# ViacheslavDanilov/oct_segmentation

Hardware: AMD Instinct MI355X
Metric: OCT frames/sec (704x704, bf16) fwd+bwd (higher is better)
Workload: dtype bf16; 1 GPU; unetplusplus/resnet101 1-class 704x704, batch 16/GPU, fwd+Dice+bwd+allreduce+Adam; global_batch=16, parallelism=dp1

## Files before the change

include/octseg.h:

```cpp
#ifndef OCTSEG_H
#define OCTSEG_H
#include <stddef.h>
#include <stdint.h>

#ifdef __cplusplus
extern "C" {
#endif

typedef enum {
  OCTSEG_OK = 0,
  OCTSEG_BAD_SHAPE = -1,
  OCTSEG_BAD_DTYPE = -2,
  OCTSEG_UNSUPPORTED_ARCH = -3,
  OCTSEG_HIP_ERROR = -4,
  OCTSEG_BAD_ARG = -5
} octseg_status;

typedef enum { OCTSEG_F32 = 0, OCTSEG_BF16 = 1, OCTSEG_F16 = 2 } octseg_dtype;

typedef struct {
  const char* arch;
  const char* encoder;
  int classes;
  int batch, height, width;
// ... 176 lines not shown

int octseg_resize_pil_u8(const uint8_t* src, int S, int H, int W, int C, uint8_t* tmp, uint8_t* dst, int oh, int ow, const int* xbounds,
                         const int* xkk, int xksize, const int* ybounds, const int* ykk, int yksize, void* stream);

int octseg_plan_set_frozen_bn(octseg_plan* plan, int on);
int octseg_plan_cam_target(const octseg_plan* plan, size_t* act_off, size_t* grad_off, int* dims);
int octseg_net_backward_seeded(octseg_plan* plan, const float* params, void* workspace, const float* dlogits, void* stream);
size_t octseg_cam_scratch_bytes(int N, int h, int w, int K);
int octseg_cam_maps(int dtype, const void* A, const void* G, int N, int h, int w, int K, int method, int S, void* scratch, float* maps,
                    float threshold, uint8_t* bin, const uint8_t* gt, int gt_h, int gt_w, const int* row_index, const int* col_index, int* counts,
                    const float* frames, const uint8_t* jet_bgr, double image_weight, uint8_t* overlay, void* stream);

int octseg_cam_overlay(const float* maps, const float* frames, const uint8_t* jet_bgr, int N, int S, double image_weight, uint8_t* overlay,
                       void* scratch, void* stream);

typedef enum { OCTSEG_LOSS_DICE = 0, OCTSEG_LOSS_BCE = 1, OCTSEG_LOSS_DICE_BCE = 2 } octseg_loss_kind;
int octseg_plan_set_loss(octseg_plan* plan, int kind);

int octseg_dice_forward(octseg_plan* plan, void* workspace, const float* logits, const float* target,
                        float* loss, long long* stats, void* stream);

int octseg_net_backward(octseg_plan* plan, const float* params, float* grads, void* workspace,
                        const float* logits, const float* target, float grad_scale, void* stream);

int octseg_net_train_step(octseg_plan* plan, const float* params, float* grads, float* buffers, void* workspace, const float* image,
                          const float* target, float* logits, float* loss, long long* stats, int normalize, const float* mean,
                          const float* stdv, float grad_scale, void* stream);
int octseg_plan_set_train_graph(octseg_plan* plan, int enable);

typedef void (*octseg_slice_cb)(void* user, int slice, size_t begin, size_t end);
int octseg_net_backward_sliced(octseg_plan* plan, const float* params, float* grads, void* workspace, const float* logits,
                               const float* target, float grad_scale, void* stream, int nslices, void* comm_stream,
                               octseg_slice_cb cb, void* user);

int octseg_optim_step(int kind, float* params, const float* grads, float* state_m, float* state_v,
                      size_t numel, float lr, float weight_decay, int step, float grad_scale,
                      void* stream);

int octseg_set_deterministic(int on);

int octseg_debug_set_stamp(unsigned long long* dev_buf);
int octseg_debug_set_serial(int on);

size_t octseg_conv2d_scratch_bytes(int dtype, int N, int H, int W, int Cin, int Cout, int R, int S);
int octseg_conv2d_forward(int dtype, const void* x, const float* w, const float* bias, void* y, int N,
                          int H, int W, int Cin, int Cout, int R, int S, int stride, int pad,
                          int transposed, void* scratch, void* stream);
int octseg_conv2d_backward_data(int dtype, const void* dy, const float* w, void* dx, int N, int H, int W,
                                int Cin, int Cout, int R, int S, int stride, int pad, int transposed,
                                void* scratch, void* stream);
int octseg_conv2d_backward_weight(int dtype, const void* x, const void* dy, float* dw, int N, int H,
                                  int W, int Cin, int Cout, int R, int S, int stride, int pad,
                                  int transposed, void* stream);

#define OCTSEG_CONV_MAX_SRC 5
typedef enum { OCTSEG_CONV_FORWARD = 0, OCTSEG_CONV_BACKWARD_DATA = 1, OCTSEG_CONV_BACKWARD_WEIGHT = 2 } octseg_conv_mode;
typedef enum { OCTSEG_ROUTE_THIN = 0, OCTSEG_ROUTE_GEMM1X1, OCTSEG_ROUTE_CONV3X3P, OCTSEG_ROUTE_MFMA16, OCTSEG_ROUTE_MFMA11,
               OCTSEG_ROUTE_MFMA_WIDEN,
               OCTSEG_ROUTE_MFMA11_MASKED, OCTSEG_ROUTE_MFMA16_MASKED } octseg_conv_route;
typedef enum { OCTSEG_WROUTE_THIN = 0, OCTSEG_WROUTE_WGRAD1X1, OCTSEG_WROUTE_CONVT16, OCTSEG_WROUTE_MFMA } octseg_wgrad_route;
typedef struct {
  const void* ptr; const float* scale; const float* shift;
  int C, H, W, up, relu;
} octseg_conv_src;
typedef struct { void* ptr; int accum, pool; } octseg_conv_dst;
typedef struct {
// ... 119 lines not shown
```

oct_segmentation_amd/_lib.py:

```python
import ctypes as C
import os

def set_hw_queues_for_collectives():
    os.environ.setdefault('GPU_MAX_HW_QUEUES', '8')


if int(os.environ.get('WORLD_SIZE', '1') or 1) > 1:
    set_hw_queues_for_collectives()

import torch

_HERE = os.path.dirname(os.path.abspath(__file__))
LIB_PATH = os.path.join(_HERE, 'liboctseg_hip.so')

F32, BF16, F16 = 0, 1, 2
P_CONV, P_CONVT, P_STEM, P_VEC = 0, 1, 2, 3
OPT_KINDS = {'SGD': 0, 'Adam': 1, 'RMSprop': 2, 'RAdam': 3}


class NetDesc(C.Structure):
    _fields_ = [('arch', C.c_char_p), ('encoder', C.c_char_p), ('classes', C.c_int), ('batch', C.c_int),
                ('height', C.c_int), ('width', C.c_int), ('dtype', C.c_int)]


# ... 117 lines not shown
    'octseg_pair_distance_counts': (C.c_int, [_P, _P] + [C.c_int] * 5 + [_P] + [C.c_int] * 3 + [_P, C.c_size_t, _P, _P, _P]),
    'octseg_pair_distance_keys': (C.c_int, [_P, _P] + [C.c_int] * 5 + [_P] + [C.c_int] * 3 + [_P, C.c_size_t, C.c_longlong, _P, _P, C.c_longlong,
                                            _P, _P]),
    'octseg_pair_distance_min': (C.c_int, [_P, _P] + [C.c_int] * 5 + [_P] + [C.c_int] * 3 + [_P, C.c_size_t, _P, _P]),
    'octseg_volume_distance_scratch_bytes': (C.c_size_t, [C.c_int] * 7),
    'octseg_volume_boundary': (C.c_int, [_P] + [C.c_int] * 4 + [_P, C.c_size_t, _P, _P]),
    'octseg_volume_distance': (C.c_int, [_P] + [C.c_int] * 6 + [_P, C.c_size_t, _P, _P]),
    'octseg_volume_pair_distance_counts': (C.c_int, [_P, _P] + [C.c_int] * 5 + [_P] + [C.c_int] * 3 + [_P, C.c_size_t, _P, _P, _P]),
    'octseg_volume_pair_distance_keys': (C.c_int, [_P, _P] + [C.c_int] * 5 + [_P] + [C.c_int] * 4 + [_P, C.c_size_t, C.c_longlong, _P, _P,
                                                   C.c_longlong, _P, _P]),
    'octseg_volume_pair_distance_min': (C.c_int, [_P, _P] + [C.c_int] * 5 + [_P] + [C.c_int] * 4 + [_P, C.c_size_t, _P, _P]),
    'octseg_signed_distance_scratch_bytes': (C.c_size_t, [C.c_int] * 4),
    'octseg_stack_signed_distance': (C.c_int, [_P] + [C.c_int] * 4 + [_P, C.c_size_t, _P, _P]),
    'octseg_signed_blend': (C.c_int, [_P] + [C.c_int] * 4 + [_P, C.c_int, _P, C.c_int, _P, _P]),
    'octseg_skeleton_scratch_bytes': (C.c_size_t, [C.c_int] * 4),
    'octseg_stack_skeleton': (C.c_int, [_P] + [C.c_int] * 5 + [_P, C.c_size_t, _P, _P, _P]),
    'octseg_prune_scratch_bytes': (C.c_size_t, [C.c_int] * 4),
    'octseg_stack_prune': (C.c_int, [_P] + [C.c_int] * 7 + [_P, C.c_size_t, _P, _P, _P]),
    'octseg_volume_normalize': (C.c_int, [_P] + [C.c_int] * 6 + [_P, _P, _P]),
    'octseg_resize_pil_u8': (C.c_int, [_P] + [C.c_int] * 4 + [_P, _P, C.c_int, C.c_int, _P, _P, C.c_int, _P, _P, C.c_int, _P]),
    'octseg_plan_set_frozen_bn': (C.c_int, [_P, C.c_int]),
    'octseg_plan_cam_target': (C.c_int, [_P, C.POINTER(C.c_size_t), C.POINTER(C.c_size_t), C.POINTER(C.c_int)]),
    'octseg_net_backward_seeded': (C.c_int, [_P, _P, _P, _P, _P]),
    'octseg_cam_scratch_bytes': (C.c_size_t, [C.c_int] * 4),
    'octseg_cam_maps': (C.c_int, [C.c_int, _P, _P] + [C.c_int] * 6 + [_P, _P, C.c_float, _P, _P, C.c_int, C.c_int, _P, _P, _P, _P, _P, C.c_double, _P, _P]),
    'octseg_cam_overlay': (C.c_int, [_P, _P, _P, C.c_int, C.c_int, C.c_double, _P, _P, _P]),
    'octseg_plan_set_loss': (C.c_int, [_P, C.c_int]),
    'octseg_dice_forward': (C.c_int, [_P, _P, _P, _P, _P, _P, _P]),
    'octseg_net_backward': (C.c_int, [_P, _P, _P, _P, _P, _P, C.c_float, _P]),
    'octseg_net_train_step': (C.c_int, [_P, _P, _P, _P, _P, _P, _P, _P, _P, _P, C.c_int, C.POINTER(C.c_float), C.POINTER(C.c_float),
                                        C.c_float, _P]),
    'octseg_plan_set_train_graph': (C.c_int, [_P, C.c_int]),
    'octseg_net_backward_sliced': (C.c_int, [_P, _P, _P, _P, _P, _P, C.c_float, _P, C.c_int, _P, SLICE_CB, _P]),
    'octseg_optim_step': (C.c_int, [C.c_int, _P, _P, _P, _P, C.c_size_t, C.c_float, C.c_float, C.c_int, C.c_float, _P]),
    'octseg_set_deterministic': (C.c_int, [C.c_int]),
    'octseg_debug_set_stamp': (C.c_int, [_P]),
    'octseg_debug_set_serial': (C.c_int, [C.c_int]),
    'octseg_conv2d_scratch_bytes': (C.c_size_t, [C.c_int] * 8),
    'octseg_conv2d_forward': (C.c_int, [C.c_int, _P, _P, _P, _P] + [C.c_int] * 10 + [_P, _P]),
    'octseg_conv2d_backward_data': (C.c_int, [C.c_int, _P, _P, _P] + [C.c_int] * 10 + [_P, _P]),
    'octseg_conv2d_backward_weight': (C.c_int, [C.c_int, _P, _P, _P] + [C.c_int] * 10 + [_P]),
    'octseg_conv_layer_op': (C.c_int, [C.c_int, C.c_int, C.POINTER(ConvLayerDesc), _P]),
    'octseg_conv_layer_route': (C.c_int, [C.c_int, C.c_int, C.POINTER(ConvLayerDesc), C.POINTER(C.c_int), C.POINTER(C.c_int)]),
    'octseg_conv_layer_slab_rows': (C.c_int, [C.c_int, C.POINTER(ConvLayerDesc), C.POINTER(C.c_int)]),
    'octseg_tied_layer_op': (C.c_int, [C.c_int, C.c_int, C.POINTER(ConvLayerDesc), C.c_int, _P]),
    'octseg_tied_layer_route': (C.c_int, [C.c_int, C.c_int, C.POINTER(ConvLayerDesc), C.c_int, C.POINTER(C.c_int), C.POINTER(C.c_int)]),
    'octseg_tied_layer_scratch_bytes': (C.c_size_t, [C.c_int, C.POINTER(ConvLayerDesc)]),
    'octseg_side_wgs': (C.c_int, []),
    'octseg_stem_op': (C.c_int, [C.c_int, C.c_int, C.POINTER(StemDesc), _P]),
    'octseg_stem_slab_rows': (C.c_int, [C.c_int] * 3),
    'octseg_sweep_op': (C.c_int, [C.c_int, C.c_int, C.POINTER(_P), C.c_int, C.POINTER(C.c_longlong), C.c_int, C.POINTER(C.c_double), C.c_int, _P]),
    'octseg_fpa_scratch_floats': (C.c_size_t, [C.c_int] * 3),
    'octseg_fpa_gscratch_floats': (C.c_size_t, [C.c_int] * 3),
    'octseg_fpa_uu_offset': (C.c_size_t, [C.c_int] * 3),
    'octseg_fpa_op': (C.c_int, [C.c_int, C.c_int, C.POINTER(FpaDesc), _P]),
    'octseg_pab_op': (C.c_int, [C.c_int, C.c_int, C.POINTER(PabDesc), _P]),
}

_lib = None


def lib():
    global _lib
    if _lib is None:
        if not os.path.exists(LIB_PATH):
            raise RuntimeError(
# ... 27 lines not shown
```

oct_segmentation_amd/csrc/api.cpp:

```cpp
#include "plan_internal.h"

#include <cctype>

using namespace octseg;
using namespace octseg::detail;

static std::string lower(const char* s) {
  std::string r(s ? s : "");
  for (auto& c : r) c = (char)tolower((unsigned char)c);
  return r;
}

template <class Outside, class Body>
static int graph_call(octseg_plan* p, bool train, bool same_key, hipGraphExec_t& exec, int& seen, hipStream_t st, Outside&& outside, Body&& body) {
  if (!same_key) {
    if (exec) { (void)hipGraphExecDestroy(exec); exec = nullptr; }
    seen = 0;
  }
  if (const int rc = outside()) return rc;
  auto replay = [&]() -> int { HIPCHK(hipGraphLaunch(exec, st)); if (train) p->packed_valid = false; return OCTSEG_OK; };
  if (exec) return replay();
  if (seen++ == 0) return body();
  if (train) p->packed_valid = false;
  hipGraph_t g = nullptr;
// ... 17 lines not shown
int octseg_version(void) { return 100; }
const char* octseg_last_error(void) { return g_err.c_str(); }

int octseg_plan_create(const octseg_net_desc* d, octseg_plan** out) {
  if (!d || !out) return fail(OCTSEG_BAD_ARG, "null argument");
  *out = nullptr;
  if (d->dtype != OCTSEG_F32 && d->dtype != OCTSEG_BF16 && d->dtype != OCTSEG_F16) return fail(OCTSEG_BAD_DTYPE, "dtype must be f32, bf16 or f16");
  if (d->height <= 0 || d->width <= 0 || d->height % 32 != 0 || d->width % 32 != 0) {
    char buf[256];
    snprintf(buf, sizeof buf, "Wrong input shape height=%d, width=%d. Expected image height and width divisible by 32.",
             d->height, d->width);
    return fail(OCTSEG_BAD_SHAPE, buf);
  }
  if (d->batch <= 0 || d->classes <= 0 || d->classes > 16) return fail(OCTSEG_BAD_SHAPE, "batch > 0 and 1 <= classes <= 16 required");
  const std::string enc = lower(d->encoder);
  if (enc != "resnet18" && enc != "resnet34" && enc != "resnet50" && enc != "resnet101" && enc != "resnet152" && enc != "timm-regnetx_002" &&
      enc != "timm-regnetx_064" && enc != "timm-regnety_120" && enc != "efficientnet-b0" && enc != "efficientnet-b5" && enc != "efficientnet-b7")
    return fail(OCTSEG_UNSUPPORTED_ARCH, "unknown encoder '" + enc + "' (resnet18 | resnet34 | resnet50 | resnet101 | resnet152 | timm-regnetx_002 | timm-regnetx_064 | timm-regnety_120 | efficientnet-b0 | efficientnet-b5 | efficientnet-b7)");
  octseg_plan* P = new octseg_plan();
  P->arch = lower(d->arch); P->encoder = enc; P->classes = d->classes;
  P->B = d->batch; P->H = d->height; P->W = d->width; P->dtype = d->dtype;
  const int rc = build_plan(P);
  if (rc) { delete P; return rc; }
  *out = P;
  return OCTSEG_OK;
}
int octseg_plan_destroy(octseg_plan* p) {
  if (p) {
    if (p->side) (void)hipStreamDestroy(p->side);
    if (p->side_bwd) (void)hipStreamDestroy(p->side_bwd);
    if (p->ev_fork) (void)hipEventDestroy(p->ev_fork);
    if (p->ev_join) (void)hipEventDestroy(p->ev_join);
    if (p->ev_slice) (void)hipEventDestroy(p->ev_slice);
    if (p->graph_exec) (void)hipGraphExecDestroy(p->graph_exec);
    if (p->tgraph_exec) (void)hipGraphExecDestroy(p->tgraph_exec);
  }
  delete p;
  return OCTSEG_OK;
}
size_t octseg_plan_workspace_bytes(const octseg_plan* p) { return p ? p->ws_bytes : 0; }
size_t octseg_plan_param_numel(const octseg_plan* p) { return p ? p->param_numel : 0; }
size_t octseg_plan_buffer_numel(const octseg_plan* p) { return p ? p->buffer_numel : 0; }
int octseg_plan_num_params(const octseg_plan* p) { return p ? (int)p->params.size() : 0; }
int octseg_plan_num_bn(const octseg_plan* p) { return p ? (int)p->bns.size() : 0; }
double octseg_plan_fwd_macs(const octseg_plan* p) { return p ? p->fwd_macs : 0.0; }
int octseg_plan_exec_macs(const octseg_plan* p, double* out3) {
  if (p == nullptr || out3 == nullptr) return OCTSEG_BAD_ARG;
  for (int k = 0; k < 3; ++k) out3[k] = p->exec_macs[k];
  return OCTSEG_OK;
}

int octseg_plan_param_info(const octseg_plan* p, int i, octseg_param_info* o) {
  if (!p || !o || i < 0 || i >= (int)p->params.size()) return fail(OCTSEG_BAD_ARG, "param index out of range");
  const ParamInfo& q = p->params[i];
  memset(o, 0, sizeof(*o));
  snprintf(o->name, sizeof o->name, "%s", q.name.c_str());
  o->kind = q.kind; o->R = q.R; o->S = q.S; o->O = q.O; o->I = q.I; o->KP = q.KP; o->offset = q.off; o->numel = q.numel;
  return OCTSEG_OK;
}
int octseg_plan_bn_info(const octseg_plan* p, int i, octseg_bn_info* o) {
  if (!p || !o || i < 0 || i >= (int)p->bns.size()) return fail(OCTSEG_BAD_ARG, "bn index out of range");
  const BNInfo& b = p->bns[i];
  memset(o, 0, sizeof(*o));
  snprintf(o->name, sizeof o->name, "%s", b.name.c_str());
  o->C = b.C; o->mean_offset = b.rm_off; o->var_offset = b.rv_off;
  return OCTSEG_OK;
// ... 366 lines not shown
  if (!p) return fail(OCTSEG_BAD_ARG, "null argument");
  if (kind < LOSS_DICE || kind > LOSS_DICE_BCE) return fail(OCTSEG_BAD_ARG, "loss kind must be 0 (dice), 1 (bce) or 2 (dice + bce)");
  if (kind != p->loss_kind && p->tgraph_exec) { (void)hipGraphExecDestroy(p->tgraph_exec); p->tgraph_exec = nullptr; p->tgraph_seen = 0; }
  p->loss_kind = kind;
  return OCTSEG_OK;
}
int octseg_plan_set_drop_connect(octseg_plan* p, const float* factors_dev) {
  if (!p) return fail(OCTSEG_BAD_ARG, "null argument");
  p->drop_connect = factors_dev;
  return OCTSEG_OK;
}
int octseg_plan_num_drop_connect(const octseg_plan* p) { return p ? (int)p->dc_rates.size() : 0; }
float octseg_plan_drop_connect_rate(const octseg_plan* p, int i) { return (p && i >= 0 && i < (int)p->dc_rates.size()) ? p->dc_rates[i] : -1.f; }
int octseg_plan_set_train_graph(octseg_plan* p, int enable) {
  if (!p) return fail(OCTSEG_BAD_ARG, "null argument");
  p->tgraph_enabled = enable != 0;
  if (!enable && p->tgraph_exec) { (void)hipGraphExecDestroy(p->tgraph_exec); p->tgraph_exec = nullptr; p->tgraph_seen = 0; }
  return OCTSEG_OK;
}

int octseg_net_backward_sliced(octseg_plan* p, const float* params, float* grads, void* workspace, const float* logits,
                               const float* target, float grad_scale, void* stream, int nslices, void* comm_stream,
                               octseg_slice_cb cb, void* user) {
  if (!p || !params || !grads || !workspace || !logits || !target || !cb) return fail(OCTSEG_BAD_ARG, "null argument");
  if (nslices < 1 || nslices > 64) return fail(OCTSEG_BAD_ARG, "1 <= nslices <= 64 required");
  if (p->dtype == OCTSEG_F16) return fail(OCTSEG_BAD_DTYPE, "f16 is a serving dtype: no backward");
  if (!comm_stream || comm_stream == stream) return fail(OCTSEG_BAD_ARG, "comm_stream must be a stream of its own");
  Exec E{p, params, grads, nullptr, (char*)workspace, (hipStream_t)stream, 1};
  SliceCtx S;
  S.n = nslices; S.comm = (hipStream_t)comm_stream; S.cb = cb; S.user = user;
  return run_backward(E, logits, target, grad_scale, &S);
}

int octseg_optim_step(int kind, float* params, const float* grads, float* m, float* v, size_t numel, float lr,
                      float wd, int step, float grad_scale, void* stream) {
  if (!params || !grads) return fail(OCTSEG_BAD_ARG, "null argument");
  if (kind < 0 || kind > 3) return fail(OCTSEG_BAD_ARG, "optimizer kind must be 0..3");
  if ((kind == 1 || kind == 3) && (!m || !v)) return fail(OCTSEG_BAD_ARG, "Adam/RAdam need both state arenas");
  if (kind == 2 && !v) return fail(OCTSEG_BAD_ARG, "RMSprop needs the second-moment arena");
  OptArgs a;
  memset(&a, 0, sizeof(a));
  a.p = params; a.g = grads; a.m = m; a.v = v; a.n = numel; a.kind = kind; a.lr = lr; a.wd = wd;
  a.beta1 = 0.9f; a.beta2 = 0.999f; a.eps = 1e-8f; a.alpha = 0.99f; a.momentum = 0.f; a.step = step; a.grad_scale = grad_scale;
  HIPCHK(launch_optim_step(a, (hipStream_t)stream));
  return OCTSEG_OK;
}

static unsigned long long* g_stamp = nullptr;
static bool g_serial = false;
int octseg_debug_set_stamp(unsigned long long* dev_buf) { g_stamp = dev_buf; return OCTSEG_OK; }
int octseg_debug_set_serial(int on) { g_serial = on != 0; g_prof_hbm = g_serial; return OCTSEG_OK; }

size_t octseg_conv2d_scratch_bytes(int dtype, int N, int H, int W, int Cin, int Cout, int R, int S) {
  (void)N; (void)H; (void)W;
  const size_t esz = dtype_size(dtype);
  const size_t rows_f = ((size_t)Cout + 127) / 128 * 128, k_f = ((size_t)Cin + 63) / 64 * 64;
  const size_t rows_d = ((size_t)Cin + 127) / 128 * 128, k_d = ((size_t)Cout + 63) / 64 * 64;
  return align_up((size_t)R * S * rows_f * k_f * esz) + align_up((size_t)R * S * rows_d * k_d * esz);
}

int octseg_conv2d_forward(int dtype, const void* x, const float* w, const float* bias, void* y, int N, int H, int W,
                          int Cin, int Cout, int R, int S, int stride, int pad, int transposed, void* scratch, void* stream) {
  if (!geom_ok(dtype, Cin, Cout, R, S, stride, transposed)) return fail(OCTSEG_BAD_SHAPE, "unsupported conv geometry");
  hipStream_t st = (hipStream_t)stream;
  const Geom g = op_geom(N, H, W, Cin, Cout, R, S, stride, pad, transposed);
  std::vector<ConvArgs> la;
// ... 82 lines not shown
```

oct_segmentation_amd/csrc/plan.h:

```cpp
#pragma once
#include <string>
#include <vector>
#include "common.h"
#include "kernels.h"
#include "../../include/octseg.h"

namespace octseg {

struct TensorInfo {
  int N, H, W, C;
  size_t off;
  size_t goff;
  bool need_grad;
  bool external;
  size_t mask_off = 0;
  int grad_alias = -1;
};

struct Value {
  int t = -1;
  int bn = -1;
};

struct ParamInfo {
// ... 59 lines not shown
              OP_DW,
              OP_GAP,
              OP_BCAST,
              OP_DROPE,
              OP_UPB,
              OP_BINPOOL,
              OP_RESIZE,
              OP_RELU,
              OP_DROP2D,
              OP_MOSAIC,
              OP_STATS,
              OP_SEGATE,
              OP_DWG,
              OP_BNX,
              OP_SEFC,
              OP_PAB,
              OP_FPA,
              OP_ADD };
struct Op {
  OpKind kind;
  int conv = -1;
  int bn = -1;
  Value y, res;
  int post = -1;
  bool relu = true;
  int in = -1, out = -1;
  int lane = 0;
  int gn = -1, up = 1;
  int ins[4] = {-1, -1, -1, -1};
  int dwp = -1, oc0 = 0, wc0 = 0;
  bool dw_first = true;
  size_t aux_off = 0;
  bool conv_bn = false;
};

}

struct octseg_plan {
  std::string arch, encoder;
  int classes, B, H, W, dtype;
  std::vector<octseg::TensorInfo> tensors;
  std::vector<octseg::ParamInfo> params;
  std::vector<octseg::BNInfo> bns;
  std::vector<octseg::ConvLayer> convs;
  std::vector<octseg::GNInfo> gns;
  std::vector<octseg::Op> ops;
  int head_up = 1;
  size_t z4_off = 0, dz4_off = 0;
  const float* stem_image = nullptr; int stem_normalize = 0; float stem_mean[3] = {0, 0, 0}, stem_std[3] = {1, 1, 1};
  const float* dropout_keep = nullptr;
  float dropout_p = 0.2f;
  size_t param_numel = 0, buffer_numel = 0;
  size_t ws_bytes = 0;
  size_t act_begin = 0, act_end = 0, grad_begin = 0, grad_end = 0;
  size_t slab_off = 0, slab_bytes = 0;
  bool has_lanes = false;
  size_t fin_part_off = 0, fin_cnt_off = 0;
  size_t pool_idx_off = 0;
  size_t tmp_off = 0, tmp_bytes = 0;
  size_t se_part_off = 0;
  int stem_pad = 3;
  const float* drop_connect = nullptr;
  std::vector<float> dc_rates;
  std::string run_error;
  struct { int w[6], b[6], bn[6]; int pool = -1; size_t scratch_off = 0, gscratch_off = 0; } fpa;
  size_t dlogits_off = 0;
  bool frozen_bn = false;
  int loss_kind = 0;
  size_t dice_off = 0;
  int col_tensor = -1;
  int stem_k = 7;
  int dlogits_C = 16;
  double fwd_macs = 0;
  double exec_macs[3] = {0, 0, 0};
  size_t tie_scratch_off = 0;
  bool packed_valid = false;
  bool packed_fold = false;
  const void* packed_buffers = nullptr;
  const void* packed_ws = nullptr;
  const void* packed_params = nullptr;
  std::vector<octseg::PackJob> pack_jobs;
  std::vector<unsigned long long> pack_prefix;
  unsigned long long pack_total = 0;
  size_t pack_tab_off = 0, pack_prefix_off = 0;
  const void* pack_tab_ws = nullptr;
  std::vector<octseg::BnEvalJob> bn_jobs;
  std::vector<unsigned> bn_prefix;
  unsigned bn_total = 0;
  size_t bn_tab_off = 0, bn_prefix_off = 0;
  hipStream_t side = nullptr;
  hipStream_t side_bwd = nullptr;
  hipEvent_t ev_fork = nullptr, ev_join = nullptr, ev_slice = nullptr;
  bool graph_enabled = false;
  int graph_seen = 0;
  hipGraphExec_t graph_exec = nullptr;
  struct GraphKey {
    const void* params; const void* buffers; const void* ws; const void* image; const void* logits; const void* stream;
    int normalize; float mean[3], stdv[3];
    bool operator==(const GraphKey& o) const {
      return params == o.params && buffers == o.buffers && ws == o.ws && image == o.image && logits == o.logits &&
             stream == o.stream && normalize == o.normalize && mean[0] == o.mean[0] && mean[1] == o.mean[1] &&
             mean[2] == o.mean[2] && stdv[0] == o.stdv[0] && stdv[1] == o.stdv[1] && stdv[2] == o.stdv[2];
    }
  } graph_key{};
  bool tgraph_enabled = false;
  int tgraph_seen = 0;
  hipGraphExec_t tgraph_exec = nullptr;
  struct TrainKey {
    const void *params, *grads, *buffers, *ws, *image, *target, *logits, *loss, *stats, *stream, *dropout, *drop_connect;
    int normalize; float mean[3], stdv[3], grad_scale;
    bool operator==(const TrainKey& o) const {
      return params == o.params && grads == o.grads && buffers == o.buffers && ws == o.ws && image == o.image && target == o.target &&
             logits == o.logits && loss == o.loss && stats == o.stats && stream == o.stream && dropout == o.dropout && drop_connect == o.drop_connect &&
             normalize == o.normalize && grad_scale == o.grad_scale && mean[0] == o.mean[0] && mean[1] == o.mean[1] &&
             mean[2] == o.mean[2] && stdv[0] == o.stdv[0] && stdv[1] == o.stdv[1] && stdv[2] == o.stdv[2];
    }
  } tgraph_key{};
};
```

oct_segmentation_amd/csrc/plan_backward.cpp:

```cpp
#include "plan_internal.h"

namespace octseg {
namespace detail {

int side_wgs() { return 144; }

static int bn_backward(Exec& E, int bn, const void* g, int mask, const void* out_mask, void* res_grad = nullptr, int res_store = 0,
                       const unsigned char* maskbits = nullptr) {
  octseg_plan* P = E.P;
  const BNInfo& b = P->bns[bn];
  const TensorInfo& t = P->tensors[b.y];
  BnBwdArgs a;
  memset(&a, 0, sizeof(a));
  a.g = g; a.y = E.act(b.y); a.out = out_mask; a.maskbits = maskbits;
  a.scale = E.bn_scale(bn); a.shift = E.bn_shift(bn); a.mean = E.bn_mean(bn); a.rstd = E.bn_rstd(bn);
  a.gamma = E.params + P->params[b.gamma].off;
  a.npix = (size_t)t.N * t.H * t.W; a.C = b.C; a.mask = mask;
  a.slab = (float*)(E.ws + P->slab_off);
  a.part = (double*)(E.ws + P->fin_part_off); a.counters = (unsigned*)(E.ws + P->fin_cnt_off);
  const int VEC = ev_vec(P->dtype);
  const int vpc = b.C / VEC;
  const int tpv = vpc >= 256 ? 1 : 256 / vpc;
  size_t rows = (a.npix + tpv - 1) / tpv;
  if (rows > 1024) rows = 1024;
  a.rows = (int)rows;
  if (E.grads) {
    a.dgamma = E.grads + P->params[b.gamma].off;
    a.dbeta = E.grads + P->params[b.beta].off;
  }
  a.coef = E.bn_coef(bn);
  a.dy = E.grad(b.y);
  a.res_grad = res_grad; a.res_store = res_store;
  E.ginit[b.y] = 1;
  const double tbytes = (double)a.npix * b.C * dtype_size(P->dtype);
  if (P->frozen_bn) {
  } else if (a.npix <= (size_t)BN_SMALL_COUNT) {
    ProfScope ps(3, tbytes * ((mask == 2 && !maskbits) ? 5 : 4), E.st, b.name + ".bwd_small");
    HIPCHK(launch_bn_bwd_small(P->dtype, a, E.st));
    return OCTSEG_OK;
  } else {
    {
      ProfScope ps(3, tbytes * ((mask == 2 && !maskbits) ? 3 : 2), E.st, b.name + ".bwd_reduce");
      HIPCHK(launch_bn_bwd_reduce(P->dtype, a, E.st));
    }
    HIPCHK(launch_bn_bwd_finalize(a, E.st));
  }
  {
    ProfScope ps(3, tbytes * (((mask == 2 && !maskbits) ? 4 : 3) + (res_grad ? (res_store ? 1 : 2) : 0)), E.st, b.name + ".bwd_apply");
    HIPCHK(launch_bn_bwd_apply(P->dtype, a, E.st));
  }
  return OCTSEG_OK;
}
// ... 225 lines not shown
  S.bounds[n] = P->param_numel;
  for (int k = 1; k < n; ++k) {
    const size_t want = P->param_numel * (size_t)k / n;
    size_t b = P->param_numel;
    for (auto& q : P->params) if (q.off >= want && q.off < b) b = q.off;
    S.bounds[k] = b;
  }
  for (int k = 1; k <= n; ++k) S.bounds[k] = std::max(S.bounds[k], S.bounds[k - 1]);
  S.last_op.assign(n, -1);
  auto touch = [&](int oi, int param) {
    if (param < 0) return;
    const size_t off = P->params[param].off;
    for (int k = 0; k < n; ++k)
      if (off >= S.bounds[k] && off < S.bounds[k + 1]) { if (S.last_op[k] < 0 || oi < S.last_op[k]) S.last_op[k] = oi; }
  };
  for (int oi = 0; oi < (int)P->ops.size(); ++oi) {
    const Op& op = P->ops[oi];
    if (op.kind == OP_CONV) { touch(oi, P->convs[op.conv].w); touch(oi, P->convs[op.conv].b); }
    else if (op.kind == OP_BN_FIN) { if (P->bns[op.bn].lazy) { touch(oi, P->bns[op.bn].gamma); touch(oi, P->bns[op.bn].beta); } }
    else if (op.kind == OP_GN) { touch(oi, P->gns[op.gn].gamma); touch(oi, P->gns[op.gn].beta); }
    else if (op.kind == OP_DW || op.kind == OP_DWG) touch(oi, op.dwp);
    else if (op.kind == OP_BNX) { touch(oi, P->bns[op.y.bn].gamma); touch(oi, P->bns[op.y.bn].beta); }
    else if (op.kind == OP_SEFC) { for (int i = 0; i < 4; ++i) touch(oi, op.ins[i]); }
    else if (op.kind == OP_FPA) {
      for (int l = 0; l < 6; ++l) { touch(oi, P->fpa.w[l]); touch(oi, P->fpa.b[l]); touch(oi, P->bns[P->fpa.bn[l]].gamma); touch(oi, P->bns[P->fpa.bn[l]].beta); }
    }
    else if (op.kind == OP_BN_ACT) {
      touch(oi, P->bns[op.y.bn].gamma); touch(oi, P->bns[op.y.bn].beta);
      if (op.res.t >= 0 && op.res.bn >= 0) { touch(oi, P->bns[op.res.bn].gamma); touch(oi, P->bns[op.res.bn].beta); }
    }
  }
}

int run_backward(Exec& E, const float* logits, const float* target, float grad_scale, SliceCtx* S) {
  octseg_plan* P = E.P;
  if (S) slice_plan(P, *S);
  auto fire = [&](int k) -> int {
    if (S->bounds[k + 1] == S->bounds[k]) return OCTSEG_OK;
    if (!P->ev_slice) HIPCHK(hipEventCreateWithFlags(&P->ev_slice, hipEventDisableTiming));
    HIPCHK(hipEventRecord(P->ev_slice, E.st));
    HIPCHK(hipStreamWaitEvent(S->comm, P->ev_slice, 0));
    if (E.wst && E.wst != E.st) {
      HIPCHK(hipEventRecord(P->ev_slice, E.wst));
      HIPCHK(hipStreamWaitEvent(S->comm, P->ev_slice, 0));
    }
    S->cb(S->user, k, S->bounds[k], S->bounds[k + 1]);
    return OCTSEG_OK;
  };
  if (E.data_only) {
    if (S || !P->frozen_bn) return fail(OCTSEG_BAD_ARG, "a data-only backward needs the plan in frozen-BatchNorm mode and takes no slices");
    for (int oi = (int)P->ops.size() - 1; oi > E.stop_op; --oi) {
      const OpKind k = P->ops[oi].kind;
      if (k == OP_GN || k == OP_DW || k == OP_DWG || k == OP_BNX || k == OP_FPA || k == OP_MERGE || k == OP_DROPE || k == OP_DROP2D)
        return fail(OCTSEG_UNSUPPORTED_ARCH, "a data-only backward of this graph is not built (" + P->arch + ")");
    }
  } else {
    HIPCHK(hipMemsetAsync(E.grads, 0, P->param_numel * sizeof(float), E.st));
  }
  HIPCHK(hipMemsetAsync(E.ws + P->fin_cnt_off, 0, 2 * 64 * sizeof(unsigned), E.st));
  E.ginit.assign(P->tensors.size(), 0);
  if (!serial_mode() && !E.data_only) {
    hipStream_t* wsp = P->tgraph_enabled ? &P->side : &P->side_bwd;
    if (!*wsp) HIPCHK(create_side_stream(wsp, !P->tgraph_enabled));
    if (!P->ev_fork) {
      HIPCHK(hipEventCreateWithFlags(&P->ev_fork, hipEventDisableTiming));
      HIPCHK(hipEventCreateWithFlags(&P->ev_join, hipEventDisableTiming));
    }
    E.wst = *wsp;
    HIPCHK(hipEventRecord(P->ev_fork, E.st));
    HIPCHK(hipStreamWaitEvent(E.wst, P->ev_fork, 0));
  }
  if (E.seed) {
    HIPCHK(launch_cam_seed(P->dtype, E.seed, E.ws + P->dlogits_off, P->B, P->classes, (size_t)P->H * P->W, P->dlogits_C, E.st));
  } else {
    const DiceArgs da = dice_args(P, E.ws, logits, target);
    HIPCHK(launch_dice_bwd(P->dtype, da, grad_scale, E.ws + P->dlogits_off, P->dlogits_C, E.st));
  }
  int rc;
  for (int oi = (int)P->ops.size() - 1; oi >= 0; --oi) {
    if (oi == E.stop_op) break;
    const Op& op = P->ops[oi];
    switch (op.kind) {
      case OP_STEM_COL: break;
      case OP_CONV: {
        const ConvLayer& L = P->convs[op.conv];
        if (L.head) rc = conv_backward(E, L, E.ws + (P->head_up > 1 ? P->dz4_off : P->dlogits_off), P->dlogits_C);
        else if (L.sliced) rc = conv_backward(E, L, (char*)E.grad(L.out) + (size_t)L.out_c0 * dtype_size(P->dtype), P->tensors[L.out].C);
        else rc = conv_backward(E, L, E.grad(L.out), L.Cout);
        if (rc) return rc;
        break;
      }
      case OP_BN_FIN: {
        const BNInfo& b = P->bns[op.bn];
        if (b.lazy) {
          rc = bn_backward(E, op.bn, E.grad(b.y), 1, nullptr);
          if (rc) return rc;
        }
        break;
      }
      case OP_BN_ACT: {
        const TensorInfo& t = P->tensors[op.out];
        const void* G = E.grad(op.out);
        const size_t n = (size_t)t.N * t.H * t.W * t.C;
        const int mask = !op.relu ? 0 : (op.post >= 0 ? 1 : 2);
        const bool fuse_res = mask == 2 && op.res.t >= 0 && op.res.bn < 0 && P->tensors[op.res.t].need_grad &&
                              E.grad(op.res.t) != G && E.grad(op.res.t) != E.grad(P->bns[op.y.bn].y);
        const unsigned char* mbits = (mask == 2 && t.mask_off) ? (const unsigned char*)(E.ws + t.mask_off) : nullptr;
        if (fuse_res) {
          const int acc = E.claim(op.res.t);
          rc = bn_backward(E, op.y.bn, G, mask, E.act(op.out), E.grad(op.res.t), acc ? 0 : 1, mbits);
        } else {
          rc = bn_backward(E, op.y.bn, G, mask, E.act(op.out), nullptr, 0, mbits);
        }
        if (rc) return rc;
// ... 234 lines not shown
        HIPCHK(launch_drop_bwd(P->dtype, E.grad(op.out), P->dropout_keep, 1.0f / (1.0f - P->dropout_p), E.grad(op.ins[0]), t.N, (size_t)t.H * t.W,
                               t.C, E.st));
        for (int i = 0; i < 4; ++i) E.ginit[op.ins[i]] = 1;
        break;
      }
      case OP_GN: {
        const TensorInfo& t = P->tensors[op.in];
        GnArgs ga = E.gn_args(op.gn);
        if (op.up > 1) {
          HIPCHK(launch_bilinear_adjoint(P->dtype, E.grad(op.out), E.grad(op.in), t.N, t.H, t.W, t.C, op.up, E.st));
          ga.g = E.grad(op.in);
        } else {
          ga.g = E.grad(op.out);
        }
        ga.dy = E.grad(op.in);
        E.ginit[op.in] = 1;
        HIPCHK(launch_gn_backward(P->dtype, ga, t.N, E.st));
        break;
      }
      case OP_UP2: {
        const TensorInfo& t = P->tensors[op.in];
        const int acc = E.claim(op.in);
        HIPCHK(launch_pool2x2_accum(P->dtype, E.grad(op.in), E.grad(op.out), t.N, t.H, t.W, t.C, acc ? 0 : 1, E.st));
        break;
      }
      case OP_MAXPOOL: {
        const TensorInfo& t = P->tensors[op.in];
        const int acc = E.claim(op.in);
        HIPCHK(launch_maxpool_bwd_idx(P->dtype, (const unsigned char*)(E.ws + P->pool_idx_off), E.grad(op.out), E.grad(op.in), t.N, t.H, t.W,
                                      t.C, acc ? 0 : 1, E.st));
        break;
      }
    }
    if (S)
      for (int k = 0; k < S->n; ++k)
        if (S->last_op[k] == oi) { rc = fire(k); if (rc) return rc; }
  }
  if (S)
    for (int k = 0; k < S->n; ++k)
      if (S->last_op[k] < 0) { rc = fire(k); if (rc) return rc; }
  if (E.wst && E.wst != E.st) {
    HIPCHK(hipEventRecord(P->ev_join, E.wst));
    HIPCHK(hipStreamWaitEvent(E.st, P->ev_join, 0));
  }
  return OCTSEG_OK;
}

}
}
```

oct_segmentation_amd/csrc/plan_internal.h:

```cpp
#pragma once
#include "plan.h"
#include "ev.h"

#include <algorithm>
#include <cstdint>
#include <cstdio>
#include <cstdlib>
#include <cstring>
#include <string>
#include <vector>

namespace octseg {
namespace detail __attribute__((visibility("hidden"))) {

extern thread_local std::string g_err;
int fail(int code, const std::string& msg);
#define HIPCHK(expr)                                                                      \
  do {                                                                                    \
    hipError_t _e = (expr);                                                               \
    if (_e != hipSuccess)                                                                 \
      return fail(OCTSEG_HIP_ERROR, std::string(#expr) + ": " + hipGetErrorString(_e));   \
  } while (0)

inline size_t align_up(size_t x, size_t a = 256) { return (x + a - 1) / a * a; }
// ... 38 lines not shown
  bool transposed, stem, head, sliced, accum_out, has_bn, has_bias;
  int R, S, stride, pad, nsrc;
  bool up0_whole_grad;
  bool skips_plain_grad;
  int Ca, Cs, Cout;
};
bool tie_eligible(const TieQuery& q);
struct TieImages {
  ConvPackInfo pk_fu, pk_du, pk_fs, pk_ds;
  bool du_masked;
  int du_taps() const { return du_masked ? 9 : 16; }
};
TieImages tie_images(int dtype, const Geom& up, const Geom& skip);
struct TieOffsets { size_t fu, du, fs, ds; };
void tie_pack_jobs(const TieImages& im, const TieOffsets& at, size_t w_off, int Cout, int Cin, int Ca, int Cs, std::vector<PackJob>& jobs,
                   std::vector<unsigned long long>& prefix, unsigned long long& total);
int side_wgs();
double layer_macs(const ConvLayer& L);
bool geom_ok(int dtype, int Cin, int Cout, int R, int S, int stride, int transposed);
Geom op_geom(int N, int H, int W, int Cin, int Cout, int R, int S, int stride, int pad, int transposed);

bool serial_mode();
hipError_t create_side_stream(hipStream_t* st, bool backward = false);

struct Exec {
  octseg_plan* P;
  const float* params;
  float* grads;
  float* buffers;
  char* ws;
  hipStream_t st;
  int train;
  hipStream_t wst = nullptr;
  const float* seed = nullptr;
  bool data_only = false;
  int stop_op = -1;
  std::vector<char> ginit;
  int claim(int t) { const int acc = ginit[t] ? 1 : 0; ginit[t] = 1; return acc; }

  void* act(int t) const { return ws + P->tensors[t].off; }
  void* grad(int t) const { return ws + P->tensors[t].goff; }
  float* ss(int bn) const { return (float*)(ws + P->bns[bn].ss_off); }
  float* bn_scale(int bn) const { return ss(bn); }
  float* bn_shift(int bn) const { return ss(bn) + P->bns[bn].C; }
  float* bn_mean(int bn) const { return ss(bn) + 2 * P->bns[bn].C; }
  float* bn_rstd(int bn) const { return ss(bn) + 3 * P->bns[bn].C; }
  float* bn_coef(int bn) const { return ss(bn) + 4 * P->bns[bn].C; }

  GnArgs gn_args(int gi) const {
    const GNInfo& g = P->gns[gi];
    const TensorInfo& t = P->tensors[g.y];
    GnArgs a;
    memset(&a, 0, sizeof(a));
    a.y = act(g.y);
    a.gamma = params + P->params[g.gamma].off; a.beta = params + P->params[g.beta].off;
    if (grads) { a.dgamma = grads + P->params[g.gamma].off; a.dbeta = grads + P->params[g.beta].off; }
    a.part = (float*)(ws + g.part_off); a.ss = (float*)(ws + g.ss_off); a.stat = (float*)(ws + g.stat_off); a.coef = (float*)(ws + g.coef_off);
    a.HW = (size_t)t.H * t.W; a.C = g.C; a.G = g.G; a.cpg = g.C / g.G; a.eps = 1e-5f;
    return a;
  }
  Geom geom(const ConvLayer& L) const {
    Geom g{L.R, L.S, L.stride, L.pad, L.transposed, L.N, L.IH, L.IW, L.Cin, L.OH, L.OW, L.Cout};
    if (L.stem) { g.R = g.S = 1; g.pad = 0; }
    return g;
  }
  int fill_srcs(const ConvLayer& L, SrcDesc* src) const {
    int c0 = 0, n = 0;
    for (auto& s : L.srcs) {
      const TensorInfo& t = P->tensors[s.v.t];
      SrcDesc d;
      d.ptr = (char*)act(s.v.t) + (size_t)s.c0 * dtype_size(P->dtype);
      d.scale = s.v.bn >= 0 ? bn_scale(s.v.bn) + s.c0 : nullptr;
      d.shift = s.v.bn >= 0 ? bn_shift(s.v.bn) + s.c0 : nullptr;
      d.C = t.C; d.c0 = c0; d.H = t.H; d.W = t.W; d.up = s.up; d.relu = s.v.bn >= 0 ? 1 : 0;
      src[n++] = d;
      c0 += s.cn ? s.cn : t.C;
    }
    return n;
  }
};

struct SliceCtx {
  int n = 0;
  hipStream_t comm = nullptr;
  octseg_slice_cb cb = nullptr;
  void* user = nullptr;
  std::vector<size_t> bounds;
  std::vector<int> last_op;
};

int build_plan(octseg_plan* P);
int pack_all_weights(Exec& E, bool fold);
int run_forward(Exec& E, const float* image, float* logits, int normalize, const float* mean, const float* stdv);
DiceArgs dice_args(const octseg_plan* P, char* ws, const float* logits, const float* target);
int run_backward(Exec& E, const float* logits, const float* target, float grad_scale, SliceCtx* S = nullptr);
int cam_target_op(const octseg_plan* P);

}
}
```

Measured before the change: 256.7 frames/s.

## Run backward ops on two lanes with dependency-derived cross-stream events

Builds a backward schedule that tracks gradient-buffer reads and writes per op and assigns ops to their forward lane, so independent backward branches run concurrently on a side stream. Cross-lane waits are placed only where a read-after-write or write-after-read hazard exists, and per-lane slab and partial buffers are used for BN finalize. The aim is to fill the GPU with concurrent branches that are otherwise serialized on one stream. The cost is extra event traffic and possible contention, and the path is skipped under train graphs, serial mode or when a lane-1 op touches the shared tmp buffer.

```diff
diff --git a/include/octseg.h b/include/octseg.h
--- a/include/octseg.h
+++ b/include/octseg.h
@@ -232,6 +232,9 @@
 int octseg_net_backward_sliced(octseg_plan* plan, const float* params, float* grads, void* workspace, const float* logits,
                                const float* target, float grad_scale, void* stream, int nslices, void* comm_stream,
                                octseg_slice_cb cb, void* user);
+
+long long octseg_plan_backward_schedule(const octseg_plan* plan, int* out, long long cap);
+const char* octseg_plan_op_name(const octseg_plan* plan, int op_index);
 
 int octseg_optim_step(int kind, float* params, const float* grads, float* state_m, float* state_v,
                       size_t numel, float lr, float weight_decay, int step, float grad_scale,
diff --git a/oct_segmentation_amd/_lib.py b/oct_segmentation_amd/_lib.py
--- a/oct_segmentation_amd/_lib.py
+++ b/oct_segmentation_amd/_lib.py
@@ -173,6 +173,8 @@
                                         C.c_float, _P]),
     'octseg_plan_set_train_graph': (C.c_int, [_P, C.c_int]),
     'octseg_net_backward_sliced': (C.c_int, [_P, _P, _P, _P, _P, _P, C.c_float, _P, C.c_int, _P, SLICE_CB, _P]),
+    'octseg_plan_backward_schedule': (C.c_longlong, [_P, C.POINTER(C.c_int), C.c_longlong]),
+    'octseg_plan_op_name': (C.c_char_p, [_P, C.c_int]),
     'octseg_optim_step': (C.c_int, [C.c_int, _P, _P, _P, _P, C.c_size_t, C.c_float, C.c_float, C.c_int, C.c_float, _P]),
     'octseg_set_deterministic': (C.c_int, [C.c_int]),
     'octseg_debug_set_stamp': (C.c_int, [_P]),
diff --git a/oct_segmentation_amd/csrc/api.cpp b/oct_segmentation_amd/csrc/api.cpp
--- a/oct_segmentation_amd/csrc/api.cpp
+++ b/oct_segmentation_amd/csrc/api.cpp
@@ -73,6 +73,7 @@
     if (p->ev_fork) (void)hipEventDestroy(p->ev_fork);
     if (p->ev_join) (void)hipEventDestroy(p->ev_join);
     if (p->ev_slice) (void)hipEventDestroy(p->ev_slice);
+    for (hipEvent_t e : p->ev_lane) if (e) (void)hipEventDestroy(e);
     if (p->graph_exec) (void)hipGraphExecDestroy(p->graph_exec);
     if (p->tgraph_exec) (void)hipGraphExecDestroy(p->tgraph_exec);
   }
@@ -505,6 +506,31 @@
   return run_backward(E, logits, target, grad_scale, &S);
 }
 
+long long octseg_plan_backward_schedule(const octseg_plan* p, int* out, long long cap) {
+  if (!p || (!out && cap > 0)) return -1;
+  std::vector<BwdStep> sched;
+  const bool lanes = backward_schedule(p, true, -1, sched);
+  long long n = 0;
+  auto put = [&](int v) { if (n < cap) out[n] = v; ++n; };
+  for (const BwdStep& s : sched) {
+    const Op& op = p->ops[s.op];
+    put(s.op); put((int)op.kind); put(op.lane); put(lanes ? s.lane : 0); put(s.res_grad);
+    put((int)s.waits.size()); put((int)s.reads.size()); put((int)s.writes.size());
+    for (int v : s.waits) put(v);
+    for (int v : s.reads) put(v);
+    for (int v : s.writes) put(v);
+  }
+  return n;
+}
+const char* octseg_plan_op_name(const octseg_plan* p, int op_index) {
+  if (!p || op_index < 0 || op_index >= (int)p->ops.size()) return nullptr;
+  const Op& op = p->ops[op_index];
+  if (op.kind == OP_CONV) return p->convs[op.conv].name.c_str();
+  if (op.kind == OP_BN_FIN) return p->bns[op.bn].name.c_str();
+  if (op.kind == OP_BN_ACT && op.y.bn >= 0) return p->bns[op.y.bn].name.c_str();
+  return "";
+}
+
 int octseg_optim_step(int kind, float* params, const float* grads, float* m, float* v, size_t numel, float lr,
                       float wd, int step, float grad_scale, void* stream) {
   if (!params || !grads) return fail(OCTSEG_BAD_ARG, "null argument");
diff --git a/oct_segmentation_amd/csrc/plan.h b/oct_segmentation_amd/csrc/plan.h
--- a/oct_segmentation_amd/csrc/plan.h
+++ b/oct_segmentation_amd/csrc/plan.h
@@ -115,6 +115,15 @@
   bool dw_first = true;
   size_t aux_off = 0;
   bool conv_bn = false;
+};
+
+struct BwdStep {
+  int op = -1;
+  int lane = 0;
+  int res_grad = -1;
+  std::vector<int> waits;
+  int signal = -1;
+  std::vector<int> reads, writes;
 };
 
 }
@@ -174,6 +183,9 @@
   hipStream_t side = nullptr;
   hipStream_t side_bwd = nullptr;
   hipEvent_t ev_fork = nullptr, ev_join = nullptr, ev_slice = nullptr;
+  std::vector<hipEvent_t> ev_lane;
+  std::vector<octseg::BwdStep> bwd_sched;
+  int bwd_lanes = -1;
   bool graph_enabled = false;
   int graph_seen = 0;
   hipGraphExec_t graph_exec = nullptr;
diff --git a/oct_segmentation_amd/csrc/plan_backward.cpp b/oct_segmentation_amd/csrc/plan_backward.cpp
--- a/oct_segmentation_amd/csrc/plan_backward.cpp
+++ b/oct_segmentation_amd/csrc/plan_backward.cpp
@@ -16,8 +16,9 @@
   a.scale = E.bn_scale(bn); a.shift = E.bn_shift(bn); a.mean = E.bn_mean(bn); a.rstd = E.bn_rstd(bn);
   a.gamma = E.params + P->params[b.gamma].off;
   a.npix = (size_t)t.N * t.H * t.W; a.C = b.C; a.mask = mask;
-  a.slab = (float*)(E.ws + P->slab_off);
-  a.part = (double*)(E.ws + P->fin_part_off); a.counters = (unsigned*)(E.ws + P->fin_cnt_off);
+  a.slab = (float*)(E.ws + P->slab_off + (size_t)E.lane * P->slab_bytes);
+  a.part = (double*)(E.ws + P->fin_part_off) + (size_t)E.lane * SLAB_PART_CAP * 2;
+  a.counters = (unsigned*)(E.ws + P->fin_cnt_off) + E.lane * 64;
   const int VEC = ev_vec(P->dtype);
   const int vpc = b.C / VEC;
   const int tpv = vpc >= 256 ? 1 : 256 / vpc;
@@ -309,15 +310,146 @@
   }
 }
 
+static int gbuf(const octseg_plan* P, int t) {
+  while (P->tensors[t].grad_alias >= 0) t = P->tensors[t].grad_alias;
+  return t;
+}
+static void bwd_sets(const octseg_plan* P, const Op& op, BwdStep& s) {
+  auto put = [&](std::vector<int>& v, int id) { if (std::find(v.begin(), v.end(), id) == v.end()) v.push_back(id); };
+  auto R = [&](int t) { if (t >= 0 && P->tensors[t].need_grad) put(s.reads, gbuf(P, t)); };
+  auto W = [&](int t) { if (t >= 0 && P->tensors[t].need_grad) put(s.writes, gbuf(P, t)); };
+  switch (op.kind) {
+    case OP_STEM_COL: case OP_STATS: break;
+    case OP_CONV: {
+      const ConvLayer& L = P->convs[op.conv];
+      if (L.head) put(s.reads, P->head_up > 1 ? BWD_BUF_DZ4 : BWD_BUF_DLOGITS);
+      else R(L.out);
+      bool any = false;
+      for (auto& sc : L.srcs) any = any || P->tensors[sc.v.t].need_grad;
+      if (!any) break;
+      if (L.tie & 2) {
+        W(L.srcs[0].v.t);
+        if (L.tie_Cs > 0) for (size_t i = 1; i < L.srcs.size(); ++i) W(L.srcs[i].v.t);
+        break;
+      }
+      Geom g{L.R, L.S, L.stride, L.pad, L.transposed, L.N, L.IH, L.IW, L.Cin, L.OH, L.OW, L.Cout};
+      if (L.stem) { g.R = g.S = 1; g.pad = 0; }
+      std::vector<ConvArgs> ld;
+      dgrad_launches(g, ld);
+      int up_src = -1;
+      for (size_t i = 0; i < L.srcs.size(); ++i) {
+        const int ti = L.srcs[i].v.t;
+        const TensorInfo& t = P->tensors[ti];
+        if (L.srcs[i].up && t.need_grad && ld.size() == 1 && ld[0].ostride == 1 && (L.IH % 2) == 0 && (L.IW % 2) == 0) W(ti);
+        else if (L.srcs[i].up) { put(s.writes, BWD_BUF_TMP); up_src = (int)i; }
+        else if (!t.need_grad) put(s.writes, BWD_BUF_TMP);
+        else W(ti);
+      }
+      if (up_src >= 0) { put(s.reads, BWD_BUF_TMP); W(L.srcs[up_src].v.t); }
+      break;
+    }
+    case OP_BN_FIN:
+      if (P->bns[op.bn].lazy) { R(P->bns[op.bn].y); W(P->bns[op.bn].y); }
+      break;
+    case OP_BN_ACT: {
+      R(op.out);
+      const int y = P->bns[op.y.bn].y;
+      W(y);
+      const int mask = !op.relu ? 0 : (op.post >= 0 ? 1 : 2);
+      const bool fuse_res = mask == 2 && op.res.t >= 0 && op.res.bn < 0 && P->tensors[op.res.t].need_grad &&
+                            gbuf(P, op.res.t) != gbuf(P, op.out) && gbuf(P, op.res.t) != gbuf(P, y);
+      if (fuse_res) { W(op.res.t); s.res_grad = op.res.t; }
+      else if (op.res.t >= 0) { if (op.res.bn >= 0) W(P->bns[op.res.bn].y); else W(op.res.t); }
+      W(op.post);
+      break;
+    }
+    case OP_BNX: R(op.out); W(op.y.t); W(op.post); break;
+    case OP_SEGATE: R(op.out); W(op.ins[0]); W(op.ins[1]); W(op.in); break;
+    case OP_ADD: R(op.out); W(op.in); W(op.ins[0]); break;
+    case OP_FPA: R(op.out); W(op.ins[0]); W(op.ins[1]); W(P->fpa.pool); W(op.in); break;
+    case OP_PAB: R(op.out); W(op.in); W(op.ins[0]); W(op.ins[1]); W(op.ins[2]); break;
+    case OP_MERGE: R(op.out); for (int i = 0; i < 4; ++i) W(op.ins[i]); break;
+    case OP_UPLOGITS: put(s.reads, BWD_BUF_DLOGITS); put(s.writes, BWD_BUF_DZ4); break;
+    default: R(op.out); W(op.in); break;
+  }
+}
+
+bool backward_schedule(const octseg_plan* P, bool lanes_wanted, int stop_op, std::vector<BwdStep>& out, int* nsignals) {
+  out.clear();
+  if (nsignals) *nsignals = 0;
+  bool lanes = lanes_wanted && P->has_lanes;
+  for (int oi = (int)P->ops.size() - 1; oi >= 0; --oi) {
+    if (oi == stop_op) break;
+    BwdStep s;
+    s.op = oi;
+    bwd_sets(P, P->ops[oi], s);
+    if (P->ops[oi].lane == 1)
+      for (const std::vector<int>* v : {&s.reads, &s.writes})
+        if (std::find(v->begin(), v->end(), BWD_BUF_TMP) != v->end()) lanes = false;
+    out.push_back(std::move(s));
+  }
+  if (!lanes) return false;
+  struct Last { int w[2] = {0, 0}, r[2] = {0, 0}; };
+  std::vector<Last> tl(P->tensors.size());
+  Last scratch[3];
+  auto last = [&](int id) -> Last& { return id >= 0 ? tl[id] : scratch[-2 - id]; };
+  std::vector<int> lane_ops[2] = {{BWD_SETUP, BWD_SETUP}, {BWD_SETUP}};
+  int seen[2] = {0, 0};
+  last(BWD_BUF_DLOGITS).w[0] = 1;
+  std::vector<char> signals(P->ops.size(), 0);
+  bool setup_signals = false;
+  for (BwdStep& s : out) {
+    const int l = s.lane = P->ops[s.op].lane, o = 1 - l;
+    int want = 0;
+    if (l == 1 && lane_ops[1].size() == 1) want = 1;
+    for (int id : s.reads) want = std::max(want, last(id).w[o]);
+    for (int id : s.writes) want = std::max(want, std::max(last(id).w[o], last(id).r[o]));
+    if (want > seen[l]) {
+      const int target = lane_ops[o][want];
+      s.waits.push_back(target);
+      if (target == BWD_SETUP) setup_signals = true; else signals[target] = 1;
+      seen[l] = want;
+    }
+    const int seq = (int)lane_ops[l].size();
+    for (int id : s.reads) last(id).r[l] = seq;
+    for (int id : s.writes) last(id).w[l] = seq;
+    lane_ops[l].push_back(s.op);
+  }
+  (void)setup_signals;
+  int ns = BWD_EV_FIRST;
+  for (BwdStep& s : out) if (signals[s.op]) s.signal = ns++;
+  if (nsignals) *nsignals = ns;
+  return true;
+}
+
 int run_backward(Exec& E, const float* logits, const float* target, float grad_scale, SliceCtx* S) {
   octseg_plan* P = E.P;
   if (S) slice_plan(P, *S);
+  bool lanes = P->has_lanes && !serial_mode() && !P->tgraph_enabled && !E.data_only && E.stop_op < 0;
+  if (lanes && P->bwd_lanes < 0) {
+    int ns = 0;
+    P->bwd_lanes = backward_schedule(P, true, -1, P->bwd_sched, &ns) ? 1 : 0;
+    P->ev_lane.assign(P->bwd_lanes ? ns : 0, nullptr);
+  }
+  lanes = lanes && P->bwd_lanes == 1;
+  const hipStream_t st0 = E.st;
+  hipStream_t lst[2] = {st0, st0};
+  struct Restore { Exec& E; hipStream_t st; ~Restore() { E.st = st; E.lane = 0; } } restore{E, st0};
+  if (lanes) {
+    if (!P->side) HIPCHK(create_side_stream(&P->side));
+    for (hipEvent_t& e : P->ev_lane) if (!e) HIPCHK(hipEventCreateWithFlags(&e, hipEventDisableTiming));
+    lst[1] = P->side;
+  }
   auto fire = [&](int k) -> int {
     if (S->bounds[k + 1] == S->bounds[k]) return OCTSEG_OK;
     if (!P->ev_slice) HIPCHK(hipEventCreateWithFlags(&P->ev_slice, hipEventDisableTiming));
-    HIPCHK(hipEventRecord(P->ev_slice, E.st));
+    HIPCHK(hipEventRecord(P->ev_slice, st0));
     HIPCHK(hipStreamWaitEvent(S->comm, P->ev_slice, 0));
-    if (E.wst && E.wst != E.st) {
+    if (lanes) {
+      HIPCHK(hipEventRecord(P->ev_slice, lst[1]));
+      HIPCHK(hipStreamWaitEvent(S->comm, P->ev_slice, 0));
+    }
+    if (E.wst && E.wst != st0) {
       HIPCHK(hipEventRecord(P->ev_slice, E.wst));
       HIPCHK(hipStreamWaitEvent(S->comm, P->ev_slice, 0));
     }
@@ -353,10 +485,17 @@
     const DiceArgs da = dice_args(P, E.ws, logits, target);
     HIPCHK(launch_dice_bwd(P->dtype, da, grad_scale, E.ws + P->dlogits_off, P->dlogits_C, E.st));
   }
+  if (lanes) HIPCHK(hipEventRecord(P->ev_lane[BWD_EV_SETUP], st0));
   int rc;
   for (int oi = (int)P->ops.size() - 1; oi >= 0; --oi) {
     if (oi == E.stop_op) break;
     const Op& op = P->ops[oi];
+    if (lanes) {
+      const BwdStep& bs = P->bwd_sched[P->ops.size() - 1 - oi];
+      E.lane = bs.lane; E.st = lst[bs.lane];
+      for (int w : bs.waits)
+        HIPCHK(hipStreamWaitEvent(E.st, P->ev_lane[w == BWD_SETUP ? BWD_EV_SETUP : P->bwd_sched[P->ops.size() - 1 - w].signal], 0));
+    }
     switch (op.kind) {
       case OP_STEM_COL: break;
       case OP_CONV: {
@@ -657,6 +796,8 @@
         break;
       }
     }
+    if (lanes && P->bwd_sched[P->ops.size() - 1 - oi].signal >= 0)
+      HIPCHK(hipEventRecord(P->ev_lane[P->bwd_sched[P->ops.size() - 1 - oi].signal], E.st));
     if (S)
       for (int k = 0; k < S->n; ++k)
         if (S->last_op[k] == oi) { rc = fire(k); if (rc) return rc; }
@@ -664,9 +805,14 @@
   if (S)
     for (int k = 0; k < S->n; ++k)
       if (S->last_op[k] < 0) { rc = fire(k); if (rc) return rc; }
-  if (E.wst && E.wst != E.st) {
+  E.st = st0; E.lane = 0;
+  if (lanes) {
+    HIPCHK(hipEventRecord(P->ev_lane[BWD_EV_JOIN], lst[1]));
+    HIPCHK(hipStreamWaitEvent(st0, P->ev_lane[BWD_EV_JOIN], 0));
+  }
+  if (E.wst && E.wst != st0) {
     HIPCHK(hipEventRecord(P->ev_join, E.wst));
-    HIPCHK(hipStreamWaitEvent(E.st, P->ev_join, 0));
+    HIPCHK(hipStreamWaitEvent(st0, P->ev_join, 0));
   }
   return OCTSEG_OK;
 }
diff --git a/oct_segmentation_amd/csrc/plan_internal.h b/oct_segmentation_amd/csrc/plan_internal.h
--- a/oct_segmentation_amd/csrc/plan_internal.h
+++ b/oct_segmentation_amd/csrc/plan_internal.h
@@ -94,6 +94,7 @@
   hipStream_t st;
   int train;
   hipStream_t wst = nullptr;
+  int lane = 0;
   const float* seed = nullptr;
   bool data_only = false;
   int stop_op = -1;
@@ -151,6 +152,11 @@
   std::vector<int> last_op;
 };
 
+constexpr int BWD_BUF_DLOGITS = -2, BWD_BUF_DZ4 = -3, BWD_BUF_TMP = -4;
+constexpr int BWD_SETUP = -1;
+constexpr int BWD_EV_SETUP = 0, BWD_EV_JOIN = 1, BWD_EV_FIRST = 2;
+bool backward_schedule(const octseg_plan* P, bool lanes_wanted, int stop_op, std::vector<BwdStep>& out, int* nsignals = nullptr);
+
 int build_plan(octseg_plan* P);
 int pack_all_weights(Exec& E, bool fold);
 int run_forward(Exec& E, const float* image, float* logits, int normalize, const float* mean, const float* stdv);
```

Measured after the change: 248.3 frames/s. 0.967x the previous value.
